# UltronAI/Depth-VO-Feat

Hardware: AMD Instinct MI355X
Metric: KITTI 256x832 stereo-seq samples/sec fwd+bwd (higher is better)
Workload: dtype f32

## Files before the change

### __graft_entry__.py

```python
import os
import subprocess
import sys

ROOT = os.path.dirname(os.path.abspath(__file__))
PKG = os.path.join(ROOT, "depth-vo-feat_amd")


def _paths():
    for p in (PKG, ROOT):
        if p not in sys.path:
            sys.path.insert(0, p)


def build():
    subprocess.run(["make", "-C", os.path.join(PKG, "csrc"), "-j4"], check=True)
    _paths()
    from dvf import lib as L
    lib = L.lib()
    assert lib.dvf_version() >= 100
    import DispNetS, PoseExpNet, PoseExpNet_sfm, inverse_warp, loss_functions, loss_functions_sfm
    import dvf.engine, dvf.steps


def smoke():
    _paths()
    import torch
    from oracle import nets as onets
    from oracle import steps as osteps
    import DispNetS
    import PoseExpNet
    from dvf.engine import FlatAdam
    from dvf.steps import unsupervise_losses
    from dvf.synthetic import synthetic_batch
    assert torch.cuda.is_available(), "smoke() needs the GPU: the product path has no CPU fallback"
    dev = torch.device("cuda:0")
    b, h, w = 1, 64, 128
    dsd = onets.fill_params(onets.dispnet_layers(), seed=1)
    psd = onets.fill_params(onets.posenet_layers(6, 6, 2, True), seed=2)
# ... 27 lines not shown
```

### depth-vo-feat_amd/csrc/conv_pipe.h

```cpp
#pragma once
#include "dvf_common.h"
#include "conv_epilogue.h"

namespace dvfp {

#ifdef DVF_TUNING
#define DVF_STAMP(a, var) do { if ((a).stamps) asm volatile("s_memtime %0\n\ts_waitcnt lgkmcnt(0)" : "=s"(var) :: "memory"); } while (0)
#define DVF_STAMP_RT(a, var) do { if ((a).stamps) asm volatile("s_memrealtime %0\n\ts_waitcnt lgkmcnt(0)" : "=s"(var) :: "memory"); } while (0)
#define DVF_STAMPS_ON 1
#else
#define DVF_STAMP(a, var) do { } while (0)
#define DVF_STAMP_RT(a, var) do { } while (0)
#define DVF_STAMPS_ON 0
#endif

typedef __attribute__((address_space(3))) void lds_void_t;

__device__ __forceinline__ __amdgpu_buffer_rsrc_t tensor_rsrc(const void *p) {
    const uint64_t v = reinterpret_cast<uint64_t>(p);
    const unsigned lo = __builtin_amdgcn_readfirstlane((unsigned)v), hi = __builtin_amdgcn_readfirstlane((unsigned)(v >> 32));
    return __builtin_amdgcn_make_buffer_rsrc(reinterpret_cast<void *>(((uint64_t)hi << 32) | lo), 0, 0x7FFFFFF0, 0x00020000);
}
constexpr unsigned OOB = 0x80000000u;
__device__ __forceinline__ float bload(__amdgpu_buffer_rsrc_t r, unsigned voff, unsigned soff) {
// ... 47 lines not shown
            while (((padded * IS) & 31) != ((SW * IS) & 31) && padded < rs + 32) padded += 4;
            if (((padded * IS) & 31) == ((SW * IS) & 31) && padded * 8 <= rs * 9) rs = padded;
        }
        g.RS = rs;
        g.PSR = (BN * g.PH * g.RS + 255) & ~255;
        g.NPI = g.PSR >> 8;
        return g;
    }
    g.RS = pipe_row_stride(IS == 2 ? 2 * g.PWH : g.PW, SW, SH, IS);
    g.PSR = (BN * g.PH * g.RS + 63) & ~63;
    g.NPI = g.PSR >> 6;
    return g;
}

template <int V> struct fvec;
template <> struct fvec<1> { typedef float type; };
template <> struct fvec<2> { typedef float type __attribute__((ext_vector_type(2))); };
template <> struct fvec<4> { typedef float type __attribute__((ext_vector_type(4))); };

constexpr int PIPE_THREADS = 384;
constexpr int PIPE_THREADS_4P = 512;
constexpr int PIPE_MAXNPI = 32;

template <int MT, int NT, int WM, int CKH, int TBU, int BLK = 0>
__global__ __launch_bounds__(PIPE_THREADS_4P) void conv_pipe_kernel(const PipeArgs a) {
    constexpr int CK = 2 * CKH, VW = CKH >= 4 ? 4 : CKH, CPG = CKH / VW, MTW = MT * WM;
    constexpr int UNITF = TBU * MTW * 64 * VW;
    typedef typename fvec<VW>::type avec;
    extern __shared__ __attribute__((aligned(16))) float smem[];
    const int stage_floats = a.SLmax + CK * a.PSRmax;
    const int tid = threadIdx.x, lane = tid & 63, nl = lane & 31, kh = lane >> 5;
    const int wave = __builtin_amdgcn_readfirstlane(tid >> 6);
    const int zper = gridDim.z / a.ncls;
    const int zc = blockIdx.z / zper, zr = blockIdx.z - zc * zper;
    const int ng = zr / a.KS, ks = zr - ng * a.KS;
    const PClass c = a.cls[zc];
    const int tX = blockIdx.x % a.tilesX, tY = blockIdx.x / a.tilesX;
    const int oy0 = tY * a.BH, ox0 = tX * a.BW, n0 = ng * a.BN;
    if (oy0 >= c.OHc || ox0 >= c.OWc) return;
    const int mb = blockIdx.y;
    const int SW = 1 << a.lsw, SH = 1 << a.lsh;
    const PipeGeo geo = pipe_geo(a.BH, a.BW, a.BN, a.IS, c.TA, TBU, SW, SH, a.x4, c.bx);
    const int RS = geo.RS, PSR = geo.PSR, PWH = geo.PWH;
    const int g_begin = (int)(((int64_t)a.NCH * ks) / a.KS), g_end = (int)(((int64_t)a.NCH * (ks + 1)) / a.KS);
    unsigned long long t_entry = 0, r_entry = 0;
    const int lin_block = (blockIdx.z * gridDim.y + blockIdx.y) * gridDim.x + blockIdx.x;
    DVF_STAMP(a, t_entry);
    DVF_STAMP_RT(a, r_entry);

    if (wave >= 4) {
// ... 4 lines not shown
        const int half = U(nprod == 2 ? 0 : (pidx & 1)), nhalf = U(nprod == 2 ? 1 : 2);
        const int NWP = U(c.SL >> 8);
        const int iy0 = U(oy0 * a.IS + c.by), ix0 = U(ox0 * a.IS + c.bx);
        const int sfl = U(stage_floats), PSRu = U(PSR), NPIu = U(geo.NPI), SLu = U(c.SL), SLmaxu = U(a.SLmax);
        const unsigned wbase = (unsigned)U((int)(c.wp_off + (unsigned)(mb * a.NCH) * (unsigned)c.SL));
        const __amdgpu_buffer_rsrc_t rs_w = tensor_rsrc(a.wp);
        auto issue_w = [&](int g, int st) __attribute__((always_inline)) {
            if (DVF_DBG(a, 2)) return;
            float *wl = smem + st * sfl;
            unsigned so = ((wbase + (unsigned)g * (unsigned)SLu) << 2) + ((unsigned)half << 10);
            float *dst = wl + (half << 8);
            for (int p = half; p < NWP; p += nhalf) {
                __builtin_amdgcn_raw_ptr_buffer_load_lds(rs_w, (lds_void_t *)dst, 16, (unsigned)lane << 4, so, 0, 0);
                so += (unsigned)nhalf << 10;
                dst += nhalf << 8;
            }
        };
        const int D = U(a.NST - 1), nchunks = U(g_end - g_begin), g0 = U(g_begin);
        auto stage_of = [&](int x) __attribute__((always_inline)) { return D == 1 ? (x & 1) : x % 3; };
        if DVF_DBG(a, 8) return;
        for (int x = 0; x < D; ++x)
            if (x < nchunks && (x & 1) == par) issue_w(g0 + x, stage_of(x));

        unsigned pvf[PIPE_MAXNPI];
        unsigned pbn4[PIPE_MAXNPI / 4];
#pragma unroll
        for (int q = 0; q < PIPE_MAXNPI / 4; ++q) pbn4[q] = 0u;
        {
            const int per_img = geo.PH * RS;
            const float inv_img = 1.0f / (float)per_img, inv_rs = 1.0f / (float)RS;
#pragma unroll
            for (int kk = 0; kk < PIPE_MAXNPI; ++kk) {
                pvf[kk] = OOB;
                if (kk < NPIu) {
                    const int p = a.x4 ? (((kk << 6) + lane) << 2) : ((kk << 6) + lane);
                    int bn = (int)((float)p * inv_img);
                    bn += (p - bn * per_img >= per_img) - (p - bn * per_img < 0);
                    const int rem = p - bn * per_img;
                    int row = (int)((float)rem * inv_rs);
                    row += (rem - row * RS >= RS) - (rem - row * RS < 0);
                    const int col = rem - row * RS;
                    int cs = col - geo.XA;
                    bool ok = (bn < a.BN) && (n0 + bn < a.N);
                    if (a.IS == 2 && !a.x4) {
                        cs = col < PWH ? 2 * col : 2 * (col - PWH) + 1;
                        ok = ok && (col < 2 * PWH);
                    }
                    if (!a.x4) ok = ok && (cs < geo.PW);
                    const int iy = iy0 + row, ix = ix0 + cs;
                    ok = ok && (iy >= 0) && (iy < a.IH) && (ix >= 0) && (ix < a.IW);
                    pvf[kk] = ok ? (unsigned)((iy * a.IW + ix) << 2) : OOB;
                    pbn4[kk >> 2] |= (ok ? (unsigned)bn : 0u) << ((kk & 3) * 8);
                }
            }
        }
        const __amdgpu_buffer_rsrc_t rs_zero = __builtin_amdgcn_make_buffer_rsrc(
            const_cast<float *>(a.wp), 0, 0, 0x00020000);
        const unsigned plane = (unsigned)U((a.IH * a.IW) << 2);
        int iseg = -1, iseg_first = 0, iseg_end = 0, segc = 0;
        __amdgpu_buffer_rsrc_t rs_in = rs_zero;
        unsigned img_cur = 0u;
        auto enter_segment = [&](int g) __attribute__((always_inline)) {
            while (g >= iseg_end) {
                ++iseg;
                iseg_first = iseg_end;
                iseg_end += (a.segC[iseg] + CK - 1) / CK;
            }
            iseg = U(iseg); iseg_first = U(iseg_first); iseg_end = U(iseg_end);
            segc = U(a.segC[iseg]);
            rs_in = tensor_rsrc(a.in[iseg]);
            const unsigned img = (unsigned)segc * plane;
            if (a.BN > 1) {
                const unsigned delta = img - img_cur;
#pragma unroll
                for (int kk = 0; kk < PIPE_MAXNPI; ++kk)
                    if (kk < NPIu) pvf[kk] = (pvf[kk] >> 31) ? OOB : pvf[kk] + ((pbn4[kk >> 2] >> ((kk & 3) * 8)) & 255u) * delta;
            }
            img_cur = img;
        };
        auto issue_p = [&](int g, int st, auto lanec, auto npc, auto exactc) __attribute__((always_inline)) {
            constexpr int LB = decltype(lanec)::value, NP = decltype(npc)::value;
            constexpr bool EXACT = decltype(exactc)::value;
            constexpr int PSH = LB == 16 ? 8 : 6;
            if (g >= iseg_end) enter_segment(g);
            const int c0 = U((g - iseg_first) * CK);
            const int nch = U(min(CK, segc - c0));
            float *dst = smem + st * sfl + SLmaxu + half * PSRu;
            unsigned soff = (unsigned)U((int)((unsigned)(n0 * segc + c0 + half) * plane));
            auto dma = [&](__amdgpu_buffer_rsrc_t r, float *d, unsigned vo, unsigned so) __attribute__((always_inline)) {
                if constexpr (LB == 16) __builtin_amdgcn_raw_ptr_buffer_load_lds(r, (lds_void_t *)d, 16, vo, so, 0, 0);
                else __builtin_amdgcn_raw_ptr_buffer_load_lds(r, (lds_void_t *)d, 4, vo, so, 0, 0);
            };
            int ci = half;
            if (DVF_DBG(a, 32)) {
                for (; ci < nch; ci += nhalf) {
#pragma unroll
                    for (int kk = 0; kk < NP; ++kk)
                        if (EXACT || kk < NPIu) dma(rs_in, dst + (kk << PSH), (unsigned)lane * LB, (unsigned)(kk << (PSH + 2)));
// ... 24 lines not shown
                DVF_STAMP(a, p0);
                if ((x & 1) == par) asm volatile("s_waitcnt vmcnt(0)" ::: "memory");
                DVF_STAMP(a, p1);
                __builtin_amdgcn_s_barrier();
                DVF_STAMP(a, p2);
                const int nx = x + D;
                if (nx < nchunks && (nx & 1) == par) {
                    issue_w(g0 + nx, stage_of(nx));
                    if (!DVF_DBG(a, 1)) issue_p(g0 + nx, stage_of(nx), lanec, npc, exactc);
                }
                DVF_STAMP(a, p3);
                w_vm += p1 - p0; w_bar += p2 - p1; w_iss += p3 - p2;
            }
        };
        auto by_np = [&](auto lanec) __attribute__((always_inline)) {
            switch (NPIu) {
                case 1: chunk_loop(lanec, integral_constant<int, 1>{}, std::true_type{}); break;
                case 2: chunk_loop(lanec, integral_constant<int, 2>{}, std::true_type{}); break;
                case 3: chunk_loop(lanec, integral_constant<int, 3>{}, std::true_type{}); break;
                case 4: chunk_loop(lanec, integral_constant<int, 4>{}, std::true_type{}); break;
                case 5: chunk_loop(lanec, integral_constant<int, 5>{}, std::true_type{}); break;
                case 6: chunk_loop(lanec, integral_constant<int, 6>{}, std::true_type{}); break;
                default:
                    if (NPIu <= 12) chunk_loop(lanec, integral_constant<int, 12>{}, std::false_type{});
                    else chunk_loop(lanec, integral_constant<int, PIPE_MAXNPI>{}, std::false_type{});
            }
        };
        if (a.x4) by_np(integral_constant<int, 16>{});
        else by_np(integral_constant<int, 4>{});
        if (DVF_STAMPS_ON && a.stamps && pidx == 0 && lane == 0) {
            a.stamps[8 * lin_block + 5] = w_vm; a.stamps[8 * lin_block + 6] = w_bar; a.stamps[8 * lin_block + 7] = w_iss;
        }
        return;
    }

    const int wm = wave % WM, wn = wave / WM;
    float *bias_lds = smem + a.NST * stage_floats;
    if (tid < 32 * MTW) {
        const int mm = mb * (32 * MTW) + tid;
        bias_lds[tid] = (a.bias && a.out_mode == OUT_FUSED && mm < a.M) ? a.bias[mm] : 0.f;
    }
    const int NU = c.NTG * CPG;
    int opy[NT], opx[NT], opn[NT];
    int bj[NT][VW];
    const int pxl = nl & (SW - 1), pyl = (nl >> a.lsw) & (SH - 1), pnl = nl >> (a.lsw + a.lsh);
#pragma unroll
    for (int i = 0; i < NT; ++i) {
        const int q = wn * NT + i, tx = q % a.TGX, tyn = q / a.TGX, ty = tyn % a.TGY, tn = tyn / a.TGY;
        const int SN = 32 >> (a.lsw + a.lsh);
        opy[i] = ty * SH + pyl;
        opx[i] = tx * SW + pxl;
        opn[i] = tn * SN + pnl;
        const int bbase = kh * PSR + (opn[i] * geo.PH + opy[i] * a.IS) * RS + (a.x4 ? geo.XA + opx[i] * a.IS : opx[i]);
#pragma unroll
        for (int j = 0; j < VW; ++j) bj[i][j] = bbase + j * 2 * PSR;
    }
    f32x16 acc[MT][NT];
    f32x16 asum[BLK ? MT : 1][BLK ? NT : 1];
#pragma unroll
    for (int m = 0; m < MT; ++m)
#pragma unroll
        for (int i = 0; i < NT; ++i)
#pragma unroll
            for (int r = 0; r < 16; ++r) {
                acc[m][i][r] = 0.f;
                if constexpr (BLK) asum[m][i][r] = 0.f;
            }

    auto consume = [&](int st, auto isc, auto tbec) {
        constexpr int IS = decltype(isc)::value, TBE = decltype(tbec)::value;
        const float *wl = smem + st * stage_floats;
        const float *patch = wl + a.SLmax;
        const float *ap = wl + (wm * MT) * 64 * VW + lane * VW;
        avec af[2][MT];
        float bf[2][TBE][NT][VW];
        int lta = 0, lcpg = 0, lk = 0;
        auto load_bj = [&](auto bufc, auto jc) {
            constexpr int buf = decltype(bufc)::value, j = decltype(jc)::value;
            const float *prow0 = patch + (lta * RS + lcpg * (2 * VW) * PSR);
#pragma unroll
            for (int i = 0; i < NT; ++i) {
                const float *prow = prow0 + bj[i][j];
                if constexpr (IS == 1) {
#pragma unroll
                    for (int u = 0; u < TBE; ++u) bf[buf][u][i][j] = prow[u];
                } else {
                    const float *prow2 = prow + PWH;
#pragma unroll
                    for (int u = 0; u < TBE; ++u) bf[buf][u][i][j] = (u & 1) ? prow2[u >> 1] : prow[u >> 1];
                }
            }
        };
        auto load_b = [&](auto bufc) {
            load_bj(bufc, std::integral_constant<int, 0>{});
            if constexpr (VW > 1) load_bj(bufc, std::integral_constant<int, 1>{});
            if constexpr (VW > 2) load_bj(bufc, std::integral_constant<int, 2>{});
            if constexpr (VW > 3) load_bj(bufc, std::integral_constant<int, 3>{});
        };
        auto load_a = [&](auto tpc, int unit, auto uc) {
            constexpr int tp = decltype(tpc)::value, u = decltype(uc)::value;
            const float *aptr = ap + unit * UNITF;
#pragma unroll
            for (int m = 0; m < MT; ++m) af[tp][m] = *reinterpret_cast<const avec *>(aptr + (u * MTW + m) * 64 * VW);
        };
        auto advance = [&]() {
// ... 43 lines not shown
        auto unit = [&](auto bufc, auto nbufc, auto pbc) {
            step(bufc, nbufc, pbc, std::integral_constant<int, 0>{});
            if constexpr (TBE > 1) step(bufc, nbufc, pbc, std::integral_constant<int, 1>{});
            if constexpr (TBE > 2) step(bufc, nbufc, pbc, std::integral_constant<int, 2>{});
            if constexpr (TBE > 3) step(bufc, nbufc, pbc, std::integral_constant<int, 3>{});
            if constexpr (TBE > 4) step(bufc, nbufc, pbc, std::integral_constant<int, 4>{});
            if constexpr (TBE > 5) step(bufc, nbufc, pbc, std::integral_constant<int, 5>{});
            if constexpr (TBE > 6) step(bufc, nbufc, pbc, std::integral_constant<int, 6>{});
            advance();
        };
        load_b(B0{});
        load_a(B0{}, 0, std::integral_constant<int, 0>{});
        advance();
        __builtin_amdgcn_sched_barrier(0);
        for (int k = 0; k < NU; k += 2) {
            unit(B0{}, B1{}, std::integral_constant<int, 0>{});
            if (k + 1 < NU) unit(B1{}, B0{}, std::integral_constant<int, TBE & 1>{});
        }
    };

    unsigned long long t_loop0 = 0, t_loop1 = 0, tb0 = 0, tb1 = 0, w_bar = 0;
    DVF_STAMP(a, t_loop0);
    if (!DVF_DBG(a, 8)) {
        int st = 0, since = 0;
        for (int g = g_begin; g < g_end; ++g) {
            DVF_STAMP(a, tb0);
            __syncthreads();
            DVF_STAMP(a, tb1);
            w_bar += tb1 - tb0;
            if (!DVF_DBG(a, 4)) {
                using TBfull = std::integral_constant<int, TBU>;
                using TBless = std::integral_constant<int, (TBU > 1 ? TBU - 1 : 1)>;
                if (a.IS == 2 && !a.x4) consume(st, std::integral_constant<int, 2>{}, TBfull{});
                else if (TBU > 1 && c.TB == TBU - 1 && !DVF_DBG(a, 64)) consume(st, std::integral_constant<int, 1>{}, TBless{});
                else consume(st, std::integral_constant<int, 1>{}, TBfull{});
            }
            if constexpr (BLK) {
                if (++since == a.blk) {
                    since = 0;
#pragma unroll
                    for (int m = 0; m < MT; ++m)
#pragma unroll
                        for (int i = 0; i < NT; ++i) {
                            asum[m][i] += acc[m][i];
#pragma unroll
                            for (int r = 0; r < 16; ++r) acc[m][i][r] = 0.f;
                        }
                }
            }
            st = (st + 1 == a.NST) ? 0 : st + 1;
        }
    }
    if constexpr (BLK) {
#pragma unroll
        for (int m = 0; m < MT; ++m)
#pragma unroll
            for (int i = 0; i < NT; ++i) acc[m][i] += asum[m][i];
    }

    DVF_STAMP(a, t_loop1);
    auto stamp_out = [&]() {
        if (DVF_STAMPS_ON && a.stamps && wave == 0) {
            unsigned long long t_end = 0, r_end = 0;
            asm volatile("s_waitcnt vmcnt(0)" ::: "memory");
            DVF_STAMP(a, t_end);
            DVF_STAMP_RT(a, r_end);
            if (lane == 0) {
                unsigned long long *o = a.stamps + 8 * lin_block;
                o[0] = t_loop0 - t_entry; o[1] = t_loop1 - t_loop0; o[2] = w_bar; o[3] = t_end - t_loop1; o[4] = r_end - r_entry;
            }
        }
    };
    if DVF_DBG(a, 16) { stamp_out(); return; }
    const int m0 = mb * (32 * MTW) + wm * (32 * MT);
    const int64_t HW = (int64_t)a.OH * a.OW;
    if (a.mask && a.out_mode == OUT_FUSED) {
        float *outp = a.out;
#pragma unroll
        for (int i = 0; i < NT; ++i) {
            const int oy = oy0 + opy[i], ox = ox0 + opx[i], n = n0 + opn[i];
            const int Y = oy * a.OS + c.py, X = ox * a.OS + c.px;
            const bool pok = (oy < c.OHc) && (ox < c.OWc) && (Y < a.OH) && (X < a.OW) && (opn[i] < a.BN) && (n < a.N);
// ... 15 lines not shown
                    if (pok && m0 + 4 * kh + ml < a.M) {
                        outp[base + (int64_t)ml * HW] = mk[m][r] > 0.f ? acc[m][i][r] : 0.f;
                    }
                }
            }
        }
        stamp_out();
        return;
    }
    store_tile<MT, NT>(
        acc, a.out + (a.out_mode == OUT_WS ? (int64_t)ks * a.ws_slice : 0), nullptr, a.out_mode, a.act, a.alpha, a.beta, m0, kh, a.M, HW,
        [&](int i, int64_t &off) __attribute__((always_inline)) {
            const int oy = oy0 + opy[i], ox = ox0 + opx[i], n = n0 + opn[i];
            const int Y = oy * a.OS + c.py, X = ox * a.OS + c.px;
            off = ((int64_t)n * a.M + m0 + 4 * kh) * HW + (int64_t)Y * a.OW + X;
            return (oy < c.OHc) && (ox < c.OWc) && (Y < a.OH) && (X < a.OW) && (opn[i] < a.BN) && (n < a.N);
        },
        [&](int ml) __attribute__((always_inline)) { return bias_lds[wm * (32 * MT) + 4 * kh + ml]; });
    stamp_out();
}

template <int MT, int NT, int WM>
int launch_pipe_family(const PipeArgs &a, int CKH, int TBU, dim3 grid, size_t lds, hipStream_t st, int threads);

template <int MT, int NT, int WM, int CKH, int TBU>
constexpr bool pipe_has_blk() {
#ifdef DVF_TUNING
    return true;
#else
    return MT == 2 && NT == 1 && WM == 1 && CKH >= 4 && TBU >= 2 && TBU <= 4;
#endif
}

template <int MT, int NT, int WM, int CKH, int TBU, int BLK>
inline int launch_pipe_blk(const PipeArgs &a, dim3 grid, size_t lds, hipStream_t st, int threads) {
    static bool big_lds = false;
    if (lds > 64 * 1024 && !big_lds) {
        if (hipFuncSetAttribute(reinterpret_cast<const void *>(&conv_pipe_kernel<MT, NT, WM, CKH, TBU, BLK>),
                                hipFuncAttributeMaxDynamicSharedMemorySize, 160 * 1024) != hipSuccess)
            return DVF_ERR_LAUNCH;
        big_lds = true;
    }
    conv_pipe_kernel<MT, NT, WM, CKH, TBU, BLK><<<grid, threads, lds, st>>>(a);
    return hipGetLastError() == hipSuccess ? DVF_OK : DVF_ERR_LAUNCH;
}

template <int MT, int NT, int WM, int CKH, int TBU>
inline int launch_pipe_one(const PipeArgs &a, dim3 grid, size_t lds, hipStream_t st, int threads) {
    if (a.blk) {
        if constexpr (pipe_has_blk<MT, NT, WM, CKH, TBU>()) return launch_pipe_blk<MT, NT, WM, CKH, TBU, 1>(a, grid, lds, st, threads);
        else return DVF_ERR_UNSUPPORTED;
    }
    return launch_pipe_blk<MT, NT, WM, CKH, TBU, 0>(a, grid, lds, st, threads);
}

template <int MT, int NT, int WM, int CKH>
inline int launch_pipe_tbu(const PipeArgs &a, int TBU, dim3 grid, size_t lds, hipStream_t st, int threads) {
    switch (TBU) {
        case 1: return launch_pipe_one<MT, NT, WM, CKH, 1>(a, grid, lds, st, threads);
        case 2: return launch_pipe_one<MT, NT, WM, CKH, 2>(a, grid, lds, st, threads);
        case 3: return launch_pipe_one<MT, NT, WM, CKH, 3>(a, grid, lds, st, threads);
        case 4: return launch_pipe_one<MT, NT, WM, CKH, 4>(a, grid, lds, st, threads);
        case 5: if constexpr (CKH <= 4 && WM == 1) return launch_pipe_one<MT, NT, WM, CKH, 5>(a, grid, lds, st, threads); else return DVF_ERR_UNSUPPORTED;
        case 7: if constexpr (CKH <= 4 && WM == 1) return launch_pipe_one<MT, NT, WM, CKH, 7>(a, grid, lds, st, threads); else return DVF_ERR_UNSUPPORTED;
        default: return DVF_ERR_UNSUPPORTED;
    }
}

#define DVF_PIPE_FAMILY(MT, NT, WM)                                                                              \
    template <>                                                                                                  \
    int launch_pipe_family<MT, NT, WM>(const PipeArgs &a, int CKH, int TBU, dim3 grid, size_t lds, hipStream_t st, int threads) { \
        switch (CKH) {                                                                                           \
            case 2: return launch_pipe_tbu<MT, NT, WM, 2>(a, TBU, grid, lds, st, threads);                                \
            case 4: return launch_pipe_tbu<MT, NT, WM, 4>(a, TBU, grid, lds, st, threads);                                \
            case 8: return launch_pipe_tbu<MT, NT, WM, 8>(a, TBU, grid, lds, st, threads);                                \
            default: return DVF_ERR_UNSUPPORTED;                                                                 \
        }                                                                                                        \
    }

}
```

### depth-vo-feat_amd/csrc/conv_pipe_host.h

```cpp
#pragma once
#include <string.h>
#include "dvf_common.h"
#include "conv_pipe.h"
#include "conv_op.h"

namespace {

using dvfp::PClass;
using dvfp::PipeArgs;
using dvfp::PipeGeo;
using dvfp::pipe_geo;
using dvfp::PIPE_MAXNPI;
using dvfp::OUT_FUSED;
using dvfp::OUT_ATOMIC;
using dvfp::OUT_WS;

struct alignas(8) PackArgsBody {
    const float *w;
    float *wp;
    int w_mode;
    int Mtot, Rtot, KK, m_base, M;
    int nseg, segC[DVF_MAX_SEGS];
    int ncls, NCH, CK, MB, VW, TBU;
    int TB[4], TA[4];
// ... 219 lines not shown
        splitk_reduce_mask_kernel<<<(unsigned)(planes * chunks), 256, 0, st>>>(ws, out, a.mask, a.KS, total, (int)HW, chunks);
        DVF_LAUNCH_CHECK();
    } else if (a.out_mode == OUT_WS) {
        splitk_reduce_kernel<<<(int)(nb > 4096 ? 4096 : nb), 256, 0, st>>>(ws, out, a.bias, a.KS, total, a.M, HW, a.act,
                                                                          a.alpha, a.beta);
        DVF_LAUNCH_CHECK();
    } else if (a.out_mode == OUT_ATOMIC && (a.bias || a.act != DVF_ACT_NONE)) {
        bias_act_kernel<<<(int)(nb > 2048 ? 2048 : nb), 256, 0, st>>>(out, a.bias, a.M, HW, total, a.act, a.alpha, a.beta);
        DVF_LAUNCH_CHECK();
    }
    if (a.out_mode == OUT_ATOMIC && a.mask)
        return dvf_act_bwd(out, a.mask, out, nullptr, a.N, a.M, (int)HW, DVF_ACT_RELU, 1.f, 0.f, 1, nullptr, 0, st);
    return DVF_OK;
}

#ifdef DVF_TUNING
constexpr size_t STAMP_MAX_BLOCKS = 16384;
unsigned long long *g_stamp_buf = nullptr;
int g_stamp_blocks = 0;
#endif
struct PipePlan {
    PipeArgs a;
    int MT, NT, WM, CKH, TBU, threads;
    size_t lds;
    dim3 grid;
    int64_t packed_floats;
    int64_t ws_floats;
    bool reduce_kpar;
    size_t pack_lds;
};

struct PipeOverride { int on, MT, NT, WM, CK, KS, BN, NST; };
inline PipeOverride pipe_override() {
    PipeOverride o{0, 0, 0, 0, 0, 0, 0, 0};
    if (const char *e = dvf_tune("DVF_PIPE_PLAN"))
        if (sscanf(e, "%d,%d,%d,%d,%d,%d,%d", &o.MT, &o.NT, &o.WM, &o.CK, &o.KS, &o.BN, &o.NST) >= 1) o.on = 1;
    return o;
}

struct PipeTiles { int lsw, lsh, TGX, TGY, TGN, BN; double cov; };
inline PipeTiles pipe_tiles(int OHc, int OWc, int N, int ntile, int BNwant, int IS, int TBmax) {
    PipeTiles best{5, 0, 1, ntile, 1, 1, 1e30};
    for (int lsn = 0; lsn <= 5; ++lsn) {
        const int SN = 1 << lsn;
        for (int lsw = 5 - lsn; lsw >= 0; --lsw) {
            const int lsh = 5 - lsn - lsw, SW = 1 << lsw, SH = 1 << lsh;
// ... 63 lines not shown
    PipeTiles tp = pipe_tiles(OHc, OWc, a.N, WN * NT, BN, a.IS, TBmax);
    if (tp.cov >= 1e30) return DVF_ERR_UNSUPPORTED;
    int64_t nblk = nblocks(tp);
    if (NT == 2 && nblk < 512 && !(ov.on && ov.NT)) {
        PipeTiles tp1 = pipe_tiles(OHc, OWc, a.N, WN * 1, BN, a.IS, TBmax);
        if (tp1.cov < 1e30) { NT = 1; tp = tp1; nblk = nblocks(tp); }
    }
    if (ov.on && ov.NT && WM == 1 && MT == 1) {
        NT = ov.NT;
        tp = pipe_tiles(OHc, OWc, a.N, WN * NT, BN, a.IS, TBmax);
        if (tp.cov >= 1e30) return DVF_ERR_UNSUPPORTED;
        nblk = nblocks(tp);
    }
    a.lsw = tp.lsw; a.lsh = tp.lsh; a.TGX = tp.TGX; a.TGY = tp.TGY; a.BN = tp.BN;
    a.BW = tp.TGX << tp.lsw; a.BH = tp.TGY << tp.lsh;
    a.tilesX = cdiv(OWc, a.BW); a.tilesY = cdiv(OHc, a.BH); a.NG = cdiv(a.N, a.BN);
    const int SW = 1 << a.lsw, SH = 1 << a.lsh, MB = 32 * MT * WM;
    auto slab = [&](int CK, int TA) { return (TA * TBU * CK * MB + 255) & ~255; };
    static const int ks_thr = dvf_tune("DVF_PIPE_KSTHR") ? atoi(dvf_tune("DVF_PIPE_KSTHR")) : 160;
    static const int ks_tgt = dvf_tune("DVF_PIPE_KSTGT") ? atoi(dvf_tune("DVF_PIPE_KSTGT")) : 256;
    const int KS0 = nblk < ks_thr ? (int)(ks_tgt / nblk) : 1;
    static const int big_lds_kb = dvf_tune("DVF_PIPE_BIGLDS_KB") ? atoi(dvf_tune("DVF_PIPE_BIGLDS_KB")) : 150;
    const size_t PIPE_LDS_BUDGET = (nblk * KS0 <= 256 ? big_lds_kb : 76) * 1024;
    struct Depth { int ok, CK, NST, PSRmax; size_t lds; };
    auto depth_for = [&](int x4) {
        Depth d{0, 0, 3, 0, 0};
        for (int i = 0; i < ncls; ++i) {
            const PipeGeo g = pipe_geo(a.BH, a.BW, a.BN, a.IS, cls[i].TA, TBU, SW, SH, x4, cls[i].bx);
            if (g.NPI > PIPE_MAXNPI) return d;
            d.PSRmax = g.PSR > d.PSRmax ? g.PSR : d.PSRmax;
        }
        auto lds_bytes = [&](int CK) { return ((size_t)d.NST * (slab(CK, TAmax) + (size_t)CK * d.PSRmax) + MB) * 4; };
        int CK = TBU >= 5 ? 8 : 16;
        while (CK > 4 && lds_bytes(CK) > PIPE_LDS_BUDGET) CK >>= 1;
        while (CK > 4 && CK / 2 >= maxc) CK >>= 1;
        if (lds_bytes(CK) > PIPE_LDS_BUDGET) {
            d.NST = 2;
            if (lds_bytes(CK) > PIPE_LDS_BUDGET && PIPE_LDS_BUDGET < 150 * 1024) {
                d.NST = 3;
                if (lds_bytes(CK) > 150 * 1024) d.NST = 2;
                if (lds_bytes(CK) > 150 * 1024) return d;
            }
        }
        if (ov.on && ov.CK) { CK = ov.CK; d.NST = 3; if (lds_bytes(CK) > 150 * 1024) d.NST = 2; }
        if (ov.on && ov.NST) d.NST = ov.NST;
        if ((CK != 4 && CK != 8 && CK != 16) || lds_bytes(CK) > 150 * 1024) return d;
        d.ok = 1; d.CK = CK; d.lds = lds_bytes(CK);
        return d;
    };
    int want_x4 = (a.IW % 4 == 0 && (a.BW * a.IS) % 4 == 0) ? 1 : 0;
    if (const char *e = dvf_tune("DVF_PIPE_X4")) want_x4 = want_x4 && atoi(e) != 0;
    const Depth d1 = depth_for(0), d4 = want_x4 ? depth_for(1) : Depth{0, 0, 3, 0, 0};
    static const bool x4_force = dvf_tune("DVF_PIPE_X4") && atoi(dvf_tune("DVF_PIPE_X4")) == 2;
    const bool use4 = d4.ok && (!d1.ok || x4_force || (d4.CK >= d1.CK && d4.NST >= d1.NST));
    const Depth dd = use4 ? d4 : d1;
    if (!dd.ok) return DVF_ERR_UNSUPPORTED;
    a.x4 = use4 ? 1 : 0;
    a.PSRmax = dd.PSRmax;
    const int CK = dd.CK, NST = dd.NST;
    a.NST = NST;
    a.SLmax = slab(CK, TAmax);
    a.NCH = 0;
    for (int s = 0; s < a.nseg; ++s) a.NCH += cdiv(a.segC[s], CK);
    const int mblocks = cdiv(a.M, MB);
    unsigned off = 0;
    for (int i = 0; i < ncls; ++i) {
        const ClassSpec &c = cls[i];
        const int SL = slab(CK, c.TA);
        a.cls[i] = PClass{c.py, c.px, c.by, c.bx, c.TA, c.TB, c.OHc, c.OWc, SL, c.TA, off};
        const int64_t nf = (int64_t)mblocks * a.NCH * SL;
        if ((int64_t)off + nf >= ((int64_t)1 << 29)) return DVF_ERR_UNSUPPORTED;
        off += (unsigned)nf;
    }
    pl.packed_floats = off;
    int KS = KS0;
// ... 6 lines not shown
    pl.reduce_kpar = KS >= 8 && (int64_t)a.OH * a.OW < ((int64_t)1 << 30);
    for (int s2 = 0; s2 < a.nseg; ++s2)
        if ((int64_t)a.N * a.segC[s2] * a.IH * a.IW * 4 >= ((int64_t)1 << 31) - 16) return DVF_ERR_UNSUPPORTED;
    pl.MT = MT; pl.NT = NT; pl.WM = WM; pl.CKH = CK / 2; pl.TBU = TBU; pl.lds = dd.lds;
    pl.pack_lds = (size_t)32 * ((CK * op.KK) | 1) * sizeof(float);
    if (pl.pack_lds > 64 * 1024) return DVF_ERR_UNSUPPORTED;
    pl.grid = dim3(a.tilesX * a.tilesY, mblocks, a.NG * KS * ncls);
    {
        const int per_chunk = CK * TAmax * TBmax;
        const int64_t kseq = (int64_t)cdiv(a.NCH, KS) * per_chunk;
        static const int blk_knob = dvf_tune("DVF_PIPE_BLK") ? atoi(dvf_tune("DVF_PIPE_BLK")) : -1;
        static const int blk_terms = dvf_tune("DVF_PIPE_BLKT") ? atoi(dvf_tune("DVF_PIPE_BLKT")) : 0;
        const bool deep = MT == 2 && NT == 1 && WM == 1 && CK >= 8 && TBU >= 2 && TBU <= 4 && kseq >= 512 &&
                          ((int64_t)pl.grid.x * pl.grid.y * pl.grid.z <= 256 || pl.lds > 76 * 1024);
        int every = blk_terms > 0 ? (blk_terms + per_chunk / 2) / per_chunk : 1;
        if (every < 1) every = 1;
        a.blk = blk_knob == 0 ? 0 : blk_knob > 0 ? blk_knob : blk_terms > 0 ? (kseq >= 384 ? every : 0) : (deep ? 1 : 0);
    }
    {
        const int64_t nblocks_total = (int64_t)pl.grid.x * pl.grid.y * pl.grid.z;
        static const bool no4p = dvf_tune("DVF_PIPE_NO4P") != nullptr;
        static const int mt1_4p = dvf_tune("DVF_PIPE_MT1_4P") ? atoi(dvf_tune("DVF_PIPE_MT1_4P")) : 1;
        pl.threads = (!no4p && (pl.lds > 76 * 1024 || nblocks_total <= 256 || (MT == 1 && mt1_4p))) ? dvfp::PIPE_THREADS_4P : dvfp::PIPE_THREADS;
    }
    return DVF_OK;
}

int launch_pipe(const PipeArgs &a, const PipePlan &pl, hipStream_t st) {
    using dvfp::launch_pipe_family;
    if (pl.WM == 2) {
        if (pl.NT != 1) return DVF_ERR_UNSUPPORTED;
        return pl.MT == 2 ? launch_pipe_family<2, 1, 2>(a, pl.CKH, pl.TBU, pl.grid, pl.lds, st, pl.threads)
                          : launch_pipe_family<1, 1, 2>(a, pl.CKH, pl.TBU, pl.grid, pl.lds, st, pl.threads);
    }
    if (pl.WM != 1) return DVF_ERR_UNSUPPORTED;
    if (pl.MT == 2 && pl.NT == 2) return DVF_ERR_UNSUPPORTED;
    if (pl.MT == 2) return launch_pipe_family<2, 1, 1>(a, pl.CKH, pl.TBU, pl.grid, pl.lds, st, pl.threads);
    if (pl.NT == 2) return launch_pipe_family<1, 2, 1>(a, pl.CKH, pl.TBU, pl.grid, pl.lds, st, pl.threads);
    return launch_pipe_family<1, 1, 1>(a, pl.CKH, pl.TBU, pl.grid, pl.lds, st, pl.threads);
}

int run_pipe(const ConvOp &op, const PipePlan &pl, const ConvIO &io, const float *packed, float *ws, int64_t ws_floats,
             hipStream_t st) {
    PipeArgs a = pl.a;
    for (int s = 0; s < a.nseg; ++s) {
        a.in[s] = io.in[s];
        if (a.x4 && (reinterpret_cast<uintptr_t>(a.in[s]) & 15)) return DVF_ERR_UNSUPPORTED;
    }
    a.wp = packed; a.bias = io.bias; a.mask = io.mask;
    const int mode = out_mode_of(op.covers, a.KS, ws, ws_floats, pl.ws_floats);
    int rc = prepare_output(a, mode, io.out, ws, st);
    if (rc) return rc;
    if (const char *e = dvf_tune("DVF_DBG")) a.dbg = atoi(e);
    a.stamps = nullptr;
#ifdef DVF_TUNING
    if (dvf_tune("DVF_STAMPS")) {
        const size_t nb = (size_t)pl.grid.x * pl.grid.y * pl.grid.z;
        if (!g_stamp_buf && hipMalloc(&g_stamp_buf, STAMP_MAX_BLOCKS * 64) != hipSuccess) return DVF_ERR_LAUNCH;
        if (nb <= STAMP_MAX_BLOCKS) {
            if (hipMemsetAsync(g_stamp_buf, 0, nb * 64, st) != hipSuccess) return DVF_ERR_LAUNCH;
            a.stamps = g_stamp_buf;
            g_stamp_blocks = (int)nb;
        }
    }
#endif
    dvf_plan_note(DVF_K_PIPE, pl.MT, pl.NT, pl.WM, 2 * pl.CKH, pl.TBU, a.KS, a.BN, a.NST, pl.threads, (int)pl.lds, mode | (a.ncls << 4) | (a.x4 << 8) | ((a.blk ? 1 : 0) << 9));
    if (dvf_tune("DVF_PIPE_DEBUG"))
        fprintf(stderr, "[pipe] M %d chunks %d N %d out %dx%d cls %d | MT %d NT %d WM %d CK %d TBU %d KS %d BN %d tile %dx%d "
                "(sub %dx%d) grid %ux%ux%u lds %zu x%d mode %d\n", a.M, a.NCH, a.N, a.OH, a.OW, a.ncls, pl.MT, pl.NT, pl.WM,
                2 * pl.CKH, pl.TBU, a.KS, a.BN, a.BH, a.BW, 1 << a.lsh, 1 << a.lsw, pl.grid.x, pl.grid.y, pl.grid.z, pl.lds, a.NST, mode);
    rc = launch_pipe(a, pl, st);
    return rc ? rc : finish_output(a, pl.reduce_kpar, ws, io.out, st);
}

PackArgs pack_job(const ConvOp &op, const PipePlan &pl, const float *w, float *packed, int *blocks) {
    const PipeArgs &a = pl.a;
    PackArgs p{};
    p.w = w; p.wp = packed; p.w_mode = op.w_mode; p.Mtot = op.Mtot; p.Rtot = op.Rtot; p.KK = op.KK;
    p.m_base = op.m_base; p.M = a.M; p.nseg = a.nseg;
    for (int s = 0; s < a.nseg; ++s) p.segC[s] = a.segC[s];
    p.ncls = op.ncls; p.NCH = a.NCH; p.CK = 2 * pl.CKH; p.MB = 32 * pl.MT * pl.WM; p.VW = pl.CKH >= 4 ? 4 : pl.CKH;
    p.TBU = pl.TBU;
    for (int c = 0; c < op.ncls; ++c) {
        p.SL[c] = a.cls[c].SL;
        p.TB[c] = op.cls[c].TB;
        p.TA[c] = op.cls[c].TA;
        p.wp_off[c] = a.cls[c].wp_off;
        for (int t = 0; t < op.cls[c].TA * op.cls[c].TB; ++t) p.tapmap[c][t] = (signed char)op.cls[c].tapmap[t];
    }
// ... 14 lines not shown
```

Baseline: 648.3.

## Add low-register conv pipe kernel variant targeting four waves per EU

New measurement: 664.9 (median of 6 runs). 2.6% higher.

```diff
diff --git a/__graft_entry__.py b/__graft_entry__.py
--- a/__graft_entry__.py
+++ b/__graft_entry__.py
@@ -14,6 +14,8 @@
 
 def build():
     subprocess.run(["make", "-C", os.path.join(PKG, "csrc"), "-j4"], check=True)
+    subprocess.run(["make", "-C", os.path.join(PKG, "csrc"), "TUNING=1", "-j4"], check=True)
+    assert os.path.exists(os.path.join(PKG, "dvf", "libdvf_hip_tuning.so"))
     _paths()
     from dvf import lib as L
     lib = L.lib()
diff --git a/depth-vo-feat_amd/csrc/conv_pipe.h b/depth-vo-feat_amd/csrc/conv_pipe.h
--- a/depth-vo-feat_amd/csrc/conv_pipe.h
+++ b/depth-vo-feat_amd/csrc/conv_pipe.h
@@ -93,10 +93,12 @@
 constexpr int PIPE_THREADS_4P = 512;
 constexpr int PIPE_MAXNPI = 32;
 
-template <int MT, int NT, int WM, int CKH, int TBU, int BLK = 0>
-__global__ __launch_bounds__(PIPE_THREADS_4P) void conv_pipe_kernel(const PipeArgs a) {
+template <int MT, int NT, int WM, int CKH, int TBU, int BLK = 0, int NPMAX = PIPE_MAXNPI>
+__global__ __launch_bounds__(PIPE_THREADS_4P) __attribute__((amdgpu_waves_per_eu(NPMAX < PIPE_MAXNPI ? 4 : 0)))
+void conv_pipe_kernel(const PipeArgs a) {
     constexpr int CK = 2 * CKH, VW = CKH >= 4 ? 4 : CKH, CPG = CKH / VW, MTW = MT * WM;
     constexpr int UNITF = TBU * MTW * 64 * VW;
+    static_assert(NPMAX >= 6 && NPMAX <= PIPE_MAXNPI, "by_np dispatches exact piece counts up to 6");
     typedef typename fvec<VW>::type avec;
     extern __shared__ __attribute__((aligned(16))) float smem[];
     const int stage_floats = a.SLmax + CK * a.PSRmax;
@@ -147,15 +149,15 @@
         for (int x = 0; x < D; ++x)
             if (x < nchunks && (x & 1) == par) issue_w(g0 + x, stage_of(x));
 
-        unsigned pvf[PIPE_MAXNPI];
-        unsigned pbn4[PIPE_MAXNPI / 4];
-#pragma unroll
-        for (int q = 0; q < PIPE_MAXNPI / 4; ++q) pbn4[q] = 0u;
+        unsigned pvf[NPMAX];
+        unsigned pbn4[(NPMAX + 3) / 4];
+#pragma unroll
+        for (int q = 0; q < (NPMAX + 3) / 4; ++q) pbn4[q] = 0u;
         {
             const int per_img = geo.PH * RS;
             const float inv_img = 1.0f / (float)per_img, inv_rs = 1.0f / (float)RS;
 #pragma unroll
-            for (int kk = 0; kk < PIPE_MAXNPI; ++kk) {
+            for (int kk = 0; kk < NPMAX; ++kk) {
                 pvf[kk] = OOB;
                 if (kk < NPIu) {
                     const int p = a.x4 ? (((kk << 6) + lane) << 2) : ((kk << 6) + lane);
@@ -198,7 +200,7 @@
             if (a.BN > 1) {
                 const unsigned delta = img - img_cur;
 #pragma unroll
-                for (int kk = 0; kk < PIPE_MAXNPI; ++kk)
+                for (int kk = 0; kk < NPMAX; ++kk)
                     if (kk < NPIu) pvf[kk] = (pvf[kk] >> 31) ? OOB : pvf[kk] + ((pbn4[kk >> 2] >> ((kk & 3) * 8)) & 255u) * delta;
             }
             img_cur = img;
@@ -269,8 +271,12 @@
                 case 5: chunk_loop(lanec, integral_constant<int, 5>{}, std::true_type{}); break;
                 case 6: chunk_loop(lanec, integral_constant<int, 6>{}, std::true_type{}); break;
                 default:
-                    if (NPIu <= 12) chunk_loop(lanec, integral_constant<int, 12>{}, std::false_type{});
-                    else chunk_loop(lanec, integral_constant<int, PIPE_MAXNPI>{}, std::false_type{});
+                    if constexpr (NPMAX > 12) {
+                        if (NPIu <= 12) chunk_loop(lanec, integral_constant<int, 12>{}, std::false_type{});
+                        else chunk_loop(lanec, integral_constant<int, NPMAX>{}, std::false_type{});
+                    } else {
+                        chunk_loop(lanec, integral_constant<int, NPMAX>{}, std::false_type{});
+                    }
             }
         };
         if (a.x4) by_np(integral_constant<int, 16>{});
@@ -289,18 +295,22 @@
     }
     const int NU = c.NTG * CPG;
     int opy[NT], opx[NT], opn[NT];
-    int bj[NT][VW];
+    constexpr bool LR = NPMAX < PIPE_MAXNPI;
+    int bj[NT][LR ? 1 : VW];
     const int pxl = nl & (SW - 1), pyl = (nl >> a.lsw) & (SH - 1), pnl = nl >> (a.lsw + a.lsh);
-#pragma unroll
-    for (int i = 0; i < NT; ++i) {
+    auto tile_pos = [&](int i, int pxv, int pyv, int pnv) __attribute__((always_inline)) {
         const int q = wn * NT + i, tx = q % a.TGX, tyn = q / a.TGX, ty = tyn % a.TGY, tn = tyn / a.TGY;
         const int SN = 32 >> (a.lsw + a.lsh);
-        opy[i] = ty * SH + pyl;
-        opx[i] = tx * SW + pxl;
-        opn[i] = tn * SN + pnl;
+        opy[i] = ty * SH + pyv;
+        opx[i] = tx * SW + pxv;
+        opn[i] = tn * SN + pnv;
+    };
+#pragma unroll
+    for (int i = 0; i < NT; ++i) {
+        tile_pos(i, pxl, pyl, pnl);
         const int bbase = kh * PSR + (opn[i] * geo.PH + opy[i] * a.IS) * RS + (a.x4 ? geo.XA + opx[i] * a.IS : opx[i]);
 #pragma unroll
-        for (int j = 0; j < VW; ++j) bj[i][j] = bbase + j * 2 * PSR;
+        for (int j = 0; j < (LR ? 1 : VW); ++j) bj[i][j] = bbase + j * 2 * PSR;
     }
     f32x16 acc[MT][NT];
     f32x16 asum[BLK ? MT : 1][BLK ? NT : 1];
@@ -324,10 +334,10 @@
         int lta = 0, lcpg = 0, lk = 0;
         auto load_bj = [&](auto bufc, auto jc) {
             constexpr int buf = decltype(bufc)::value, j = decltype(jc)::value;
-            const float *prow0 = patch + (lta * RS + lcpg * (2 * VW) * PSR);
+            const float *prow0 = patch + (lta * RS + (lcpg * (2 * VW) + (LR ? 2 * j : 0)) * PSR);
 #pragma unroll
             for (int i = 0; i < NT; ++i) {
-                const float *prow = prow0 + bj[i][j];
+                const float *prow = prow0 + bj[i][LR ? 0 : j];
                 if constexpr (IS == 1) {
 #pragma unroll
                     for (int u = 0; u < TBE; ++u) bf[buf][u][i][j] = prow[u];
@@ -417,33 +427,53 @@
     unsigned long long t_loop0 = 0, t_loop1 = 0, tb0 = 0, tb1 = 0, w_bar = 0;
     DVF_STAMP(a, t_loop0);
     if (!DVF_DBG(a, 8)) {
-        int st = 0, since = 0;
-        for (int g = g_begin; g < g_end; ++g) {
-            DVF_STAMP(a, tb0);
-            __syncthreads();
-            DVF_STAMP(a, tb1);
-            w_bar += tb1 - tb0;
-            if (!DVF_DBG(a, 4)) {
-                using TBfull = std::integral_constant<int, TBU>;
-                using TBless = std::integral_constant<int, (TBU > 1 ? TBU - 1 : 1)>;
-                if (a.IS == 2 && !a.x4) consume(st, std::integral_constant<int, 2>{}, TBfull{});
-                else if (TBU > 1 && c.TB == TBU - 1 && !DVF_DBG(a, 64)) consume(st, std::integral_constant<int, 1>{}, TBless{});
-                else consume(st, std::integral_constant<int, 1>{}, TBfull{});
-            }
-            if constexpr (BLK) {
-                if (++since == a.blk) {
-                    since = 0;
-#pragma unroll
-                    for (int m = 0; m < MT; ++m)
-#pragma unroll
-                        for (int i = 0; i < NT; ++i) {
-                            asum[m][i] += acc[m][i];
-#pragma unroll
-                            for (int r = 0; r < 16; ++r) acc[m][i][r] = 0.f;
-                        }
-                }
-            }
-            st = (st + 1 == a.NST) ? 0 : st + 1;
+        using IS1 = std::integral_constant<int, 1>;
+        using IS2 = std::integral_constant<int, 2>;
+        using TBfull = std::integral_constant<int, TBU>;
+        using TBless = std::integral_constant<int, (TBU > 1 ? TBU - 1 : 1)>;
+        if constexpr (LR) {
+            static_assert(!BLK, "the low-register form has no second accumulator set");
+            auto chunks = [&](auto isc, auto tbec) __attribute__((always_inline)) {
+                int st = 0;
+                for (int g = g_begin; g < g_end; ++g) {
+                    DVF_STAMP(a, tb0);
+                    __syncthreads();
+                    DVF_STAMP(a, tb1);
+                    w_bar += tb1 - tb0;
+                    if (!DVF_DBG(a, 4)) consume(st, isc, tbec);
+                    st = (st + 1 == a.NST) ? 0 : st + 1;
+                }
+            };
+            if (a.IS == 2 && !a.x4) chunks(IS2{}, TBfull{});
+            else if (TBU > 1 && c.TB == TBU - 1 && !DVF_DBG(a, 64)) chunks(IS1{}, TBless{});
+            else chunks(IS1{}, TBfull{});
+        } else {
+            int st = 0, since = 0;
+            for (int g = g_begin; g < g_end; ++g) {
+                DVF_STAMP(a, tb0);
+                __syncthreads();
+                DVF_STAMP(a, tb1);
+                w_bar += tb1 - tb0;
+                if (!DVF_DBG(a, 4)) {
+                    if (a.IS == 2 && !a.x4) consume(st, IS2{}, TBfull{});
+                    else if (TBU > 1 && c.TB == TBU - 1 && !DVF_DBG(a, 64)) consume(st, IS1{}, TBless{});
+                    else consume(st, IS1{}, TBfull{});
+                }
+                if constexpr (BLK) {
+                    if (++since == a.blk) {
+                        since = 0;
+#pragma unroll
+                        for (int m = 0; m < MT; ++m)
+#pragma unroll
+                            for (int i = 0; i < NT; ++i) {
+                                asum[m][i] += acc[m][i];
+#pragma unroll
+                                for (int r = 0; r < 16; ++r) acc[m][i][r] = 0.f;
+                            }
+                    }
+                }
+                st = (st + 1 == a.NST) ? 0 : st + 1;
+            }
         }
     }
     if constexpr (BLK) {
@@ -453,6 +483,12 @@
             for (int i = 0; i < NT; ++i) acc[m][i] += asum[m][i];
     }
 
+    if constexpr (LR) {
+        int nlv = nl;
+        asm volatile("" : "+v"(nlv));
+#pragma unroll
+        for (int i = 0; i < NT; ++i) tile_pos(i, nlv & (SW - 1), (nlv >> a.lsw) & (SH - 1), nlv >> (a.lsw + a.lsh));
+    }
     DVF_STAMP(a, t_loop1);
     auto stamp_out = [&]() {
         if (DVF_STAMPS_ON && a.stamps && wave == 0) {
@@ -514,6 +550,16 @@
 
 template <int MT, int NT, int WM>
 int launch_pipe_family(const PipeArgs &a, int CKH, int TBU, dim3 grid, size_t lds, hipStream_t st, int threads);
+template <int MT, int NT, int WM>
+int launch_pipe_family_lr(const PipeArgs &a, int CKH, int TBU, dim3 grid, size_t lds, hipStream_t st, int threads);
+
+constexpr int PIPE_LR_NPI = 12;
+constexpr size_t PIPE_LR_LDS = 80 * 1024;
+constexpr bool pipe_has_lr(int MT, int NT, int WM, int CKH, int TBU) {
+    if (WM != 1) return false;
+    if (MT == 2) return NT == 1;
+    return !(NT == 2 && CKH == 4 && TBU >= 5);
+}
 
 template <int MT, int NT, int WM, int CKH, int TBU>
 constexpr bool pipe_has_blk() {
@@ -524,50 +570,61 @@
 #endif
 }
 
-template <int MT, int NT, int WM, int CKH, int TBU, int BLK>
+template <int MT, int NT, int WM, int CKH, int TBU, int BLK, int NPMAX = PIPE_MAXNPI>
 inline int launch_pipe_blk(const PipeArgs &a, dim3 grid, size_t lds, hipStream_t st, int threads) {
     static bool big_lds = false;
     if (lds > 64 * 1024 && !big_lds) {
-        if (hipFuncSetAttribute(reinterpret_cast<const void *>(&conv_pipe_kernel<MT, NT, WM, CKH, TBU, BLK>),
+        if (hipFuncSetAttribute(reinterpret_cast<const void *>(&conv_pipe_kernel<MT, NT, WM, CKH, TBU, BLK, NPMAX>),
                                 hipFuncAttributeMaxDynamicSharedMemorySize, 160 * 1024) != hipSuccess)
             return DVF_ERR_LAUNCH;
         big_lds = true;
     }
-    conv_pipe_kernel<MT, NT, WM, CKH, TBU, BLK><<<grid, threads, lds, st>>>(a);
+    conv_pipe_kernel<MT, NT, WM, CKH, TBU, BLK, NPMAX><<<grid, threads, lds, st>>>(a);
     return hipGetLastError() == hipSuccess ? DVF_OK : DVF_ERR_LAUNCH;
 }
 
-template <int MT, int NT, int WM, int CKH, int TBU>
+template <int MT, int NT, int WM, int CKH, int TBU, bool LR>
 inline int launch_pipe_one(const PipeArgs &a, dim3 grid, size_t lds, hipStream_t st, int threads) {
-    if (a.blk) {
-        if constexpr (pipe_has_blk<MT, NT, WM, CKH, TBU>()) return launch_pipe_blk<MT, NT, WM, CKH, TBU, 1>(a, grid, lds, st, threads);
-        else return DVF_ERR_UNSUPPORTED;
-    }
-    return launch_pipe_blk<MT, NT, WM, CKH, TBU, 0>(a, grid, lds, st, threads);
-}
-
-template <int MT, int NT, int WM, int CKH>
+    if constexpr (LR) {
+        if constexpr (pipe_has_lr(MT, NT, WM, CKH, TBU)) {
+            if (a.blk || lds > PIPE_LR_LDS) return DVF_ERR_UNSUPPORTED;
+            return launch_pipe_blk<MT, NT, WM, CKH, TBU, 0, PIPE_LR_NPI>(a, grid, lds, st, threads);
+        } else {
+            return DVF_ERR_UNSUPPORTED;
+        }
+    } else {
+        if (a.blk) {
+            if constexpr (pipe_has_blk<MT, NT, WM, CKH, TBU>()) return launch_pipe_blk<MT, NT, WM, CKH, TBU, 1>(a, grid, lds, st, threads);
+            else return DVF_ERR_UNSUPPORTED;
+        }
+        return launch_pipe_blk<MT, NT, WM, CKH, TBU, 0>(a, grid, lds, st, threads);
+    }
+}
+
+template <int MT, int NT, int WM, int CKH, bool LR>
 inline int launch_pipe_tbu(const PipeArgs &a, int TBU, dim3 grid, size_t lds, hipStream_t st, int threads) {
     switch (TBU) {
-        case 1: return launch_pipe_one<MT, NT, WM, CKH, 1>(a, grid, lds, st, threads);
-        case 2: return launch_pipe_one<MT, NT, WM, CKH, 2>(a, grid, lds, st, threads);
-        case 3: return launch_pipe_one<MT, NT, WM, CKH, 3>(a, grid, lds, st, threads);
-        case 4: return launch_pipe_one<MT, NT, WM, CKH, 4>(a, grid, lds, st, threads);
-        case 5: if constexpr (CKH <= 4 && WM == 1) return launch_pipe_one<MT, NT, WM, CKH, 5>(a, grid, lds, st, threads); else return DVF_ERR_UNSUPPORTED;
-        case 7: if constexpr (CKH <= 4 && WM == 1) return launch_pipe_one<MT, NT, WM, CKH, 7>(a, grid, lds, st, threads); else return DVF_ERR_UNSUPPORTED;
+        case 1: return launch_pipe_one<MT, NT, WM, CKH, 1, LR>(a, grid, lds, st, threads);
+        case 2: return launch_pipe_one<MT, NT, WM, CKH, 2, LR>(a, grid, lds, st, threads);
+        case 3: return launch_pipe_one<MT, NT, WM, CKH, 3, LR>(a, grid, lds, st, threads);
+        case 4: return launch_pipe_one<MT, NT, WM, CKH, 4, LR>(a, grid, lds, st, threads);
+        case 5: if constexpr (CKH <= 4 && WM == 1) return launch_pipe_one<MT, NT, WM, CKH, 5, LR>(a, grid, lds, st, threads); else return DVF_ERR_UNSUPPORTED;
+        case 7: if constexpr (CKH <= 4 && WM == 1) return launch_pipe_one<MT, NT, WM, CKH, 7, LR>(a, grid, lds, st, threads); else return DVF_ERR_UNSUPPORTED;
         default: return DVF_ERR_UNSUPPORTED;
     }
 }
 
-#define DVF_PIPE_FAMILY(MT, NT, WM)                                                                              \
+#define DVF_PIPE_FAMILY_(NAME, LR, MT, NT, WM)                                                                   \
     template <>                                                                                                  \
-    int launch_pipe_family<MT, NT, WM>(const PipeArgs &a, int CKH, int TBU, dim3 grid, size_t lds, hipStream_t st, int threads) { \
+    int NAME<MT, NT, WM>(const PipeArgs &a, int CKH, int TBU, dim3 grid, size_t lds, hipStream_t st, int threads) { \
         switch (CKH) {                                                                                           \
-            case 2: return launch_pipe_tbu<MT, NT, WM, 2>(a, TBU, grid, lds, st, threads);                                \
-            case 4: return launch_pipe_tbu<MT, NT, WM, 4>(a, TBU, grid, lds, st, threads);                                \
-            case 8: return launch_pipe_tbu<MT, NT, WM, 8>(a, TBU, grid, lds, st, threads);                                \
+            case 2: return launch_pipe_tbu<MT, NT, WM, 2, LR>(a, TBU, grid, lds, st, threads);                   \
+            case 4: return launch_pipe_tbu<MT, NT, WM, 4, LR>(a, TBU, grid, lds, st, threads);                   \
+            case 8: return launch_pipe_tbu<MT, NT, WM, 8, LR>(a, TBU, grid, lds, st, threads);                   \
             default: return DVF_ERR_UNSUPPORTED;                                                                 \
         }                                                                                                        \
     }
-
-}
+#define DVF_PIPE_FAMILY(MT, NT, WM) DVF_PIPE_FAMILY_(launch_pipe_family, false, MT, NT, WM)
+#define DVF_PIPE_FAMILY_LR(MT, NT, WM) DVF_PIPE_FAMILY_(launch_pipe_family_lr, true, MT, NT, WM)
+
+}
diff --git a/depth-vo-feat_amd/csrc/conv_pipe_host.h b/depth-vo-feat_amd/csrc/conv_pipe_host.h
--- a/depth-vo-feat_amd/csrc/conv_pipe_host.h
+++ b/depth-vo-feat_amd/csrc/conv_pipe_host.h
@@ -265,6 +265,8 @@
 struct PipePlan {
     PipeArgs a;
     int MT, NT, WM, CKH, TBU, threads;
+    int npi;
+    int lr;
     size_t lds;
     dim3 grid;
     int64_t packed_floats;
@@ -374,13 +376,14 @@
     const int KS0 = nblk < ks_thr ? (int)(ks_tgt / nblk) : 1;
     static const int big_lds_kb = dvf_tune("DVF_PIPE_BIGLDS_KB") ? atoi(dvf_tune("DVF_PIPE_BIGLDS_KB")) : 150;
     const size_t PIPE_LDS_BUDGET = (nblk * KS0 <= 256 ? big_lds_kb : 76) * 1024;
-    struct Depth { int ok, CK, NST, PSRmax; size_t lds; };
+    struct Depth { int ok, CK, NST, PSRmax; size_t lds; int NPImax; };
     auto depth_for = [&](int x4) {
-        Depth d{0, 0, 3, 0, 0};
+        Depth d{0, 0, 3, 0, 0, 0};
         for (int i = 0; i < ncls; ++i) {
             const PipeGeo g = pipe_geo(a.BH, a.BW, a.BN, a.IS, cls[i].TA, TBU, SW, SH, x4, cls[i].bx);
             if (g.NPI > PIPE_MAXNPI) return d;
             d.PSRmax = g.PSR > d.PSRmax ? g.PSR : d.PSRmax;
+            d.NPImax = g.NPI > d.NPImax ? g.NPI : d.NPImax;
         }
         auto lds_bytes = [&](int CK) { return ((size_t)d.NST * (slab(CK, TAmax) + (size_t)CK * d.PSRmax) + MB) * 4; };
         int CK = TBU >= 5 ? 8 : 16;
@@ -402,7 +405,7 @@
     };
     int want_x4 = (a.IW % 4 == 0 && (a.BW * a.IS) % 4 == 0) ? 1 : 0;
     if (const char *e = dvf_tune("DVF_PIPE_X4")) want_x4 = want_x4 && atoi(e) != 0;
-    const Depth d1 = depth_for(0), d4 = want_x4 ? depth_for(1) : Depth{0, 0, 3, 0, 0};
+    const Depth d1 = depth_for(0), d4 = want_x4 ? depth_for(1) : Depth{0, 0, 3, 0, 0, 0};
     static const bool x4_force = dvf_tune("DVF_PIPE_X4") && atoi(dvf_tune("DVF_PIPE_X4")) == 2;
     const bool use4 = d4.ok && (!d1.ok || x4_force || (d4.CK >= d1.CK && d4.NST >= d1.NST));
     const Depth dd = use4 ? d4 : d1;
@@ -455,12 +458,23 @@
         static const bool no4p = dvf_tune("DVF_PIPE_NO4P") != nullptr;
         static const int mt1_4p = dvf_tune("DVF_PIPE_MT1_4P") ? atoi(dvf_tune("DVF_PIPE_MT1_4P")) : 1;
         pl.threads = (!no4p && (pl.lds > 76 * 1024 || nblocks_total <= 256 || (MT == 1 && mt1_4p))) ? dvfp::PIPE_THREADS_4P : dvfp::PIPE_THREADS;
+        pl.npi = dd.NPImax;
+        const bool lr_fits = !a.blk && dd.NPImax <= dvfp::PIPE_LR_NPI && pl.lds <= dvfp::PIPE_LR_LDS &&
+                             dvfp::pipe_has_lr(MT, NT, WM, CK / 2, TBU);
+        pl.lr = lr_fits && nblocks_total > 256;
+        if (const char *e = dvf_tune("DVF_PIPE_LR")) pl.lr = lr_fits && atoi(e) != 0;
     }
     return DVF_OK;
 }
 
 int launch_pipe(const PipeArgs &a, const PipePlan &pl, hipStream_t st) {
     using dvfp::launch_pipe_family;
+    if (pl.lr) {
+        if (pl.WM != 1) return DVF_ERR_UNSUPPORTED;
+        if (pl.MT == 2) return dvfp::launch_pipe_family_lr<2, 1, 1>(a, pl.CKH, pl.TBU, pl.grid, pl.lds, st, pl.threads);
+        return pl.NT == 2 ? dvfp::launch_pipe_family_lr<1, 2, 1>(a, pl.CKH, pl.TBU, pl.grid, pl.lds, st, pl.threads)
+                          : dvfp::launch_pipe_family_lr<1, 1, 1>(a, pl.CKH, pl.TBU, pl.grid, pl.lds, st, pl.threads);
+    }
     if (pl.WM == 2) {
         if (pl.NT != 1) return DVF_ERR_UNSUPPORTED;
         return pl.MT == 2 ? launch_pipe_family<2, 1, 2>(a, pl.CKH, pl.TBU, pl.grid, pl.lds, st, pl.threads)
@@ -497,7 +511,7 @@
         }
     }
 #endif
-    dvf_plan_note(DVF_K_PIPE, pl.MT, pl.NT, pl.WM, 2 * pl.CKH, pl.TBU, a.KS, a.BN, a.NST, pl.threads, (int)pl.lds, mode | (a.ncls << 4) | (a.x4 << 8) | ((a.blk ? 1 : 0) << 9));
+    dvf_plan_note(DVF_K_PIPE, pl.MT, pl.NT, pl.WM, 2 * pl.CKH, pl.TBU, a.KS, a.BN, a.NST, pl.threads, (int)pl.lds, mode | (a.ncls << 4) | (a.x4 << 8) | ((a.blk ? 1 : 0) << 9) | (pl.lr << 10) | (pl.npi << 11));
     if (dvf_tune("DVF_PIPE_DEBUG"))
         fprintf(stderr, "[pipe] M %d chunks %d N %d out %dx%d cls %d | MT %d NT %d WM %d CK %d TBU %d KS %d BN %d tile %dx%d "
                 "(sub %dx%d) grid %ux%ux%u lds %zu x%d mode %d\n", a.M, a.NCH, a.N, a.OH, a.OW, a.ncls, pl.MT, pl.NT, pl.WM,
diff --git a/depth-vo-feat_amd/csrc/conv_pipe_inst_d.hip b/depth-vo-feat_amd/csrc/conv_pipe_inst_d.hip
--- /dev/null
+++ b/depth-vo-feat_amd/csrc/conv_pipe_inst_d.hip
@@ -0,0 +1,5 @@
+#include "conv_pipe.h"
+namespace dvfp {
+DVF_PIPE_FAMILY_LR(1, 1, 1)
+DVF_PIPE_FAMILY_LR(1, 2, 1)
+}
diff --git a/depth-vo-feat_amd/csrc/conv_pipe_inst_e.hip b/depth-vo-feat_amd/csrc/conv_pipe_inst_e.hip
--- /dev/null
+++ b/depth-vo-feat_amd/csrc/conv_pipe_inst_e.hip
@@ -0,0 +1,4 @@
+#include "conv_pipe.h"
+namespace dvfp {
+DVF_PIPE_FAMILY_LR(2, 1, 1)
+}
```
